# samedii/perceptor

Measured on AMD Instinct MI355X. Metric: denoising steps/sec (UNet+CLIP-grad) at 512x512 batch 8, higher is better.
Workload: dtype bf16

## Files before the change

perceptor_amd/csrc/attn.hip:

```cpp
#include "common.h"
#include "../../include/perceptor_hip.h"

namespace {

__device__ __forceinline__ int64_t tfrag(int bh, int ntb, int tb, int ks, int db, int lhi, int l31) {
  return ((((((int64_t)bh * ntb + tb) * 2 + ks) * 2 + db) * 2 + lhi) * 32 + l31) * 8;
}

__device__ __forceinline__ int64_t rfrag(int bh, int ntb, int tb, int kk, int lhi, int l31) {
  return ((((((int64_t)bh * ntb + tb) * 4 + kk) * 2 + lhi) * 32 + l31) * 8);
}

template <typename T_>
__global__ __launch_bounds__(256) void qkv_split_kernel(const u16* __restrict__ qkv, u16* __restrict__ q,
                                                        u16* __restrict__ k, u16* __restrict__ vt, int T, int Tp,
                                                        int heads, int order) {
  __shared__ u16 sv[32][72];
  const int tid = threadIdx.x, t0 = blockIdx.x * 32, bh = blockIdx.y;
  const int n = bh / heads, h = bh - n * heads;
  const int C = heads * 64;
  const int qoff = order == 0 ? h * 192 : h * 64;
  const int koff = order == 0 ? h * 192 + 64 : C + h * 64;
  const int voff = order == 0 ? h * 192 + 128 : 2 * C + h * 64;
  const int row = tid >> 3, ch = tid & 7;
  const int t = t0 + row;
  uint4 vq = make_uint4(0, 0, 0, 0), vk = vq, vv = vq;
  if (t < T) {
    const u16* src = qkv + ((int64_t)n * T + t) * 3 * C + ch * 8;
    vq = *(const uint4*)(src + qoff); vk = *(const uint4*)(src + koff); vv = *(const uint4*)(src + voff);
  }
  const int64_t o = rfrag(bh, Tp >> 5, blockIdx.x, ch >> 1, ch & 1, row);
  *(uint4*)(q + o) = vq;
  *(uint4*)(k + o) = vk;
  *(uint4*)(&sv[row][ch * 8]) = vv;
  __syncthreads();
  const int d = tid >> 2, tc = tid & 3, fks = tc >> 1, flhi = tc & 1;
  u16 e[8];
#pragma unroll
  for (int j = 0; j < 8; ++j) e[j] = sv[16 * fks + 4 * flhi + (j & 3) + 8 * (j >> 2)][d];
  uint4 out = make_uint4(e[0] | (e[1] << 16), e[2] | (e[3] << 16), e[4] | (e[5] << 16), e[6] | (e[7] << 16));
  *(uint4*)(vt + tfrag(bh, Tp >> 5, blockIdx.x, fks, d >> 5, flhi, d & 31)) = out;
}

__device__ __forceinline__ void head_xcd_remap(int& bx, int& bh) {
// ... 420 lines not shown
    u16* ovp = okp + C;
#pragma unroll
    for (int g = 0; g < 4; ++g) {
      *(uint2*)(okp + 8 * g) = pack4<T_>(dk0[4 * g], dk0[4 * g + 1], dk0[4 * g + 2], dk0[4 * g + 3]);
      *(uint2*)(okp + 32 + 8 * g) = pack4<T_>(dk1[4 * g], dk1[4 * g + 1], dk1[4 * g + 2], dk1[4 * g + 3]);
      *(uint2*)(ovp + 8 * g) = pack4<T_>(dv0[4 * g], dv0[4 * g + 1], dv0[4 * g + 2], dv0[4 * g + 3]);
      *(uint2*)(ovp + 32 + 8 * g) = pack4<T_>(dv1[4 * g], dv1[4 * g + 1], dv1[4 * g + 2], dv1[4 * g + 3]);
    }
  }
}

template <typename T_>
__global__ __launch_bounds__(64) void vit_attn_bwd_kernel(const u16* __restrict__ q, const u16* __restrict__ k, const u16* __restrict__ v,
                                                          const u16* __restrict__ qt, const u16* __restrict__ kt,
                                                          const u16* __restrict__ d_o, const u16* __restrict__ d_ot,
                                                          const float* __restrict__ lse, const float* __restrict__ delta,
                                                          u16* __restrict__ dqkv, int T, int Tp, int heads, float scale) {
  int bx, bh;
  head_xcd_remap(bx, bh);
  if (blockIdx.z == 0) vit_attn_dkdv_body<T_>(q, k, v, qt, d_o, d_ot, lse, delta, dqkv, T, Tp, heads, scale, bx, bh);
  else vit_attn_dq_body<T_>(q, k, v, kt, d_o, lse, delta, dqkv, T, Tp, heads, scale, bx, bh);
}

}

#define VIT_BY_DTYPE(KERN, G, B, ...)                                                             \
  do {                                                                                            \
    if (dtype == PMI_DT_BF16) hipLaunchKernelGGL(KERN<BF16>, G, B, 0, (hipStream_t)s, __VA_ARGS__); \
    else hipLaunchKernelGGL(KERN<F16>, G, B, 0, (hipStream_t)s, __VA_ARGS__);                     \
  } while (0)

extern "C" int pmi_vit_attn_fwd(const void* qkv, void* ws16, float* lse, void* out, int N, int T, int heads, float scale, int dtype,
                                pmi_stream_t s) {
  if (!qkv || !ws16 || !lse || !out || N <= 0 || T <= 0 || heads <= 0) return PMI_ERR_ARG;
  const int Tp = (T + 31) / 32 * 32;
  const int64_t blk = (int64_t)N * heads * Tp * 64;
  u16* w = (u16*)ws16;
  dim3 g(Tp / 32, N * heads);
  VIT_BY_DTYPE(vit_qkv_split_kernel, g, dim3(256), (const u16*)qkv, w, w + blk, w + 2 * blk, w + 3 * blk, w + 4 * blk, w + 5 * blk, T, Tp, heads);
  PMI_CHECK_LAUNCH();
  VIT_BY_DTYPE(vit_attn_fwd_kernel, g, dim3(64), w, w + blk, w + 5 * blk, (u16*)out, lse, T, Tp, heads, scale);
  PMI_CHECK_LAUNCH();
  return PMI_OK;
}

extern "C" int pmi_vit_attn_bwd(const void* ws16, const float* lse, const void* o, const void* dout, void* ws16b, float* delta,
                                void* dqkv, int N, int T, int heads, float scale, int dtype, pmi_stream_t s) {
  if (!ws16 || !lse || !o || !dout || !ws16b || !delta || !dqkv || N <= 0 || T <= 0 || heads <= 0) return PMI_ERR_ARG;
  const int Tp = (T + 31) / 32 * 32;
  const int64_t blk = (int64_t)N * heads * Tp * 64;
  const u16* w = (const u16*)ws16;
  u16* wb = (u16*)ws16b;
  dim3 g(Tp / 32, N * heads);
  VIT_BY_DTYPE(vit_do_prep_kernel, g, dim3(256), (const u16*)dout, (const u16*)o, wb, wb + blk, delta, T, Tp, heads);
  PMI_CHECK_LAUNCH();
  dim3 g2(Tp / 32, N * heads, 2);
  VIT_BY_DTYPE(vit_attn_bwd_kernel, g2, dim3(64), w, w + blk, w + 2 * blk, w + 3 * blk, w + 4 * blk, wb, wb + blk, lse, delta, (u16*)dqkv, T, Tp,
               heads, scale);
  PMI_CHECK_LAUNCH();
  return PMI_OK;
}
```

perceptor_amd/csrc/common.h:

```cpp
#pragma once
#include <type_traits>
#include <hip/hip_runtime.h>
#include <stdint.h>

#define PMI_OK 0
#define PMI_ERR_ARG (-1)
#define PMI_ERR_LAUNCH (-2)

#define PMI_DT_F16 0
#define PMI_DT_BF16 1
#define PMI_DT_F16X2 2

#define PMI_ACT_NONE 0
#define PMI_ACT_RELU 1
#define PMI_ACT_SILU 2
#define PMI_ACT_GELU 3
#define PMI_ACT_QUICKGELU 4
#define PMI_ACT_GEGLU 5

typedef _Float16 f16x8 __attribute__((ext_vector_type(8)));
typedef __bf16 bf16x8 __attribute__((ext_vector_type(8)));
typedef float f32x2 __attribute__((ext_vector_type(2)));
typedef _Float16 f16x2 __attribute__((ext_vector_type(2)));
typedef __bf16 bf16x2 __attribute__((ext_vector_type(2)));
// ... 138 lines not shown
  act_switch(act, [&](auto act_c) __attribute__((always_inline)) {
#pragma unroll
    for (int e = 0; e < N; ++e) v[e] = act_apply(v[e], decltype(act_c)::value);
  });
}

__device__ __forceinline__ float act_grad(float x, int act) {
  switch (act) {
    case PMI_ACT_RELU: return x > 0.f ? 1.f : 0.f;
    case PMI_ACT_SILU: { const float s = 1.f / (1.f + __expf(-x)); return s * (1.f + x * (1.f - s)); }
    case PMI_ACT_GELU: return 0.5f * (1.f + fast_erff(x * 0.70710678118654752f)) + x * 0.3989422804014327f * __expf(-0.5f * x * x);
    case PMI_ACT_QUICKGELU: { const float s = 1.f / (1.f + __expf(-1.702f * x)); return s * (1.f + 1.702f * x * (1.f - s)); }
    default: return 1.f;
  }
}

__device__ __forceinline__ float wave_sum(float v) {
#pragma unroll
  for (int o = 32; o > 0; o >>= 1) v += __shfl_xor(v, o);
  return v;
}
__device__ __forceinline__ float wave_max(float v) {
#pragma unroll
  for (int o = 32; o > 0; o >>= 1) v = fmaxf(v, __shfl_xor(v, o));
  return v;
}

__device__ __forceinline__ int xcd_remap(int bid, int nwg) {
  const int q = nwg >> 3, r = nwg & 7, xcd = bid & 7, idx = bid >> 3;
  const int base = xcd < r ? xcd * (q + 1) : r * (q + 1) + (xcd - r) * q;
  return base + idx;
}

#define PMI_CHECK_LAUNCH()                                   \
  do {                                                       \
    hipError_t e__ = hipGetLastError();                      \
    if (e__ != hipSuccess) return PMI_ERR_LAUNCH;            \
  } while (0)
```

perceptor_amd/csrc/gemm_wd.hip:

```cpp
#include "common.h"
#include "../../include/perceptor_hip.h"

namespace {

template <typename T, int MB, bool TWO = false, int NWV = 8, bool CONV = false>
__global__ __launch_bounds__(NWV * 64, 2) void gemm_wd_kernel(const pmi_igemm_args a) {
  constexpr int TM = 16 * MB, BN = NWV * 32, BK = 128, NT = NWV * 64;
  constexpr int ROW = 2 * BK + 32;
  constexpr int TILE = TM * ROW;
  constexpr int NPI = (TM * 16 + NT - 1) / NT;
  constexpr int HIMG = TM * (BN * 2 + 16);
  __shared__ __attribute__((aligned(16))) char smem[2 * TILE > 2 * HIMG ? 2 * TILE : 2 * HIMG];

  const int tid = threadIdx.x, lane = tid & 63;
  const int wid = __builtin_amdgcn_readfirstlane(tid >> 6);
#ifdef PMI_STAMPS
#define GSTAMP(k) do { if (tid == 0 && a.reserved == 77 && a.splitk <= 1) ((long long*)a.ws)[(int64_t)blockIdx.x * 8 + (k)] = (long long)wall_clock64(); } while (0)
#else
#define GSTAMP(k) do {} while (0)
#endif
  GSTAMP(0);
  const int tiles_n = (a.N + BN - 1) / BN, tiles_m = (a.M + TM - 1) / TM;
  const int logical = xcd_remap(blockIdx.x, tiles_m * tiles_n);
  const bool mfast = (int64_t)a.M <= (int64_t)a.N;
  const int tm = mfast ? logical % tiles_m : logical / tiles_n, tn = mfast ? logical / tiles_m : logical % tiles_n;
  const int m0 = tm * TM, n0 = tn * BN;
  const int nch_all = (a.K + BK - 1) / BK;
  int c0 = 0, nch = nch_all;
  if (a.splitk > 1) {
    const int per = (nch_all + a.splitk - 1) / a.splitk;
    c0 = blockIdx.z * per;
    nch = min(per, nch_all - c0);
  }

  const int rows = min(TM, a.M - m0);
  const int K0 = TWO ? a.C0 : a.K;
  const int64_t mb_ = CONV ? 0 : m0, mr_ = CONV ? a.M : rows;
  const __amdgpu_buffer_rsrc_t rsrc_a = make_rsrc((const u16*)a.A0 + mb_ * a.lda0, ((mr_ - 1) * a.lda0 + K0) * 2);
// ... 84 lines not shown
  for (int mb = 0; mb < MB; ++mb) xf[mb] = *(const uint4*)(smem + frag0 + mb * 16 * ROW);

  for (int chunk = 0; chunk < nch; ++chunk) {
    const char* const pb = smem + (chunk & 1) * TILE;
    char* const pn = smem + ((chunk + 1) & 1) * TILE;
    const bool more2 = chunk + 2 < nch;
#pragma unroll
    for (int s = 0; s < 4; ++s) {
      load_w((s + 3) & 3, chunk * 4 + s + 3);
      if (s == 2) store_tile(pn);
      if (s == 3) {
        load_tile(more2 ? chunk + 2 : chunk, more2);
        __syncthreads();
      }
      __builtin_amdgcn_sched_barrier(0);
      const char* const nb = (s < 3 ? pb + (s + 1) * 64 : pn) + frag0;
#pragma unroll
      for (int mb = 0; mb < MB; ++mb) {
        acc[mb][0] = T::mfma16(wq[s][0], xf[mb], acc[mb][0]);
        acc[mb][1] = T::mfma16(wq[s][1], xf[mb], acc[mb][1]);
        xf[mb] = *(const uint4*)(nb + mb * 16 * ROW);
      }
#pragma unroll
      for (int mb = 0; mb < MB; ++mb) {
        __builtin_amdgcn_sched_group_barrier(0x008, 2, 0);
        __builtin_amdgcn_sched_group_barrier(0x100, 1, 0);
      }
      __builtin_amdgcn_sched_barrier(0);
    }
  }
  __syncthreads();
  GSTAMP(2);

  const bool raw = a.splitk > 1;
  if (a.act == PMI_ACT_GEGLU) {
    constexpr int GROW = (BN / 2) * 2 + 16;
    const int cl = wid * 16 + 4 * (lane >> 4);
    float4 bv = make_float4(0.f, 0.f, 0.f, 0.f), bg = bv;
    if (a.bias && wave_live) { bv = *(const float4*)(a.bias + n0 + wid * 32 + 4 * (lane >> 4)); bg = *(const float4*)(a.bias + n0 + wid * 32 + 16 + 4 * (lane >> 4)); }
#pragma unroll
    for (int mb = 0; mb < MB; ++mb) {
      const f32x4 cv = acc[mb][0], cg = acc[mb][1];
      float v[4] = {cv[0] * a.alpha + bv.x, cv[1] * a.alpha + bv.y, cv[2] * a.alpha + bv.z, cv[3] * a.alpha + bv.w};
      const float g[4] = {cg[0] * a.alpha + bg.x, cg[1] * a.alpha + bg.y, cg[2] * a.alpha + bg.z, cg[3] * a.alpha + bg.w};
#pragma unroll
      for (int e = 0; e < 4; ++e) v[e] *= act_apply(g[e], PMI_ACT_GELU);
      *(uint2*)(smem + (mb * 16 + (lane & 15)) * GROW + cl * 2) = pack4<T>(v[0], v[1], v[2], v[3]);
    }
    __syncthreads();
    const int gc8 = tid % (BN / 16), grow = tid / (BN / 16);
    const int nh = a.N >> 1, nh0 = n0 >> 1;
#pragma unroll
    for (int j = 0; j < (TM + 31) / 32; ++j) {
      const int r = grow + 32 * j, m = m0 + r;
      if (r >= TM || m >= a.M || nh0 + gc8 * 8 >= nh) continue;
      *(uint4*)((u16*)a.D + (int64_t)m * a.ldd + nh0 + gc8 * 8) = *(const uint4*)(smem + r * GROW + gc8 * 16);
    }
    GSTAMP(3);
    return;
  }
  if (!raw && !a.out_f32 && !(a.R && a.res_f32)) {
    constexpr int HROW = BN * 2 + 16;
    static_assert(2 * TM * HROW <= 160 * 1024, "the two 16-bit epilogue images (output, pre-activation) must fit the LDS");
    act_switch(a.act, [&](auto act_c) __attribute__((always_inline)) {
      constexpr int ACT = decltype(act_c)::value;
#pragma unroll
// ... 79 lines not shown
      const int m = m0 + mb * 16 + (lane & 15);
      if (m >= a.M) continue;
      const f32x4 c = acc[mb][cb];
      if (raw) {
        *(float4*)(Dslab + (int64_t)m * a.N + n) = make_float4(c[0], c[1], c[2], c[3]);
        continue;
      }
      float v[4] = {c[0] * a.alpha + bv.x, c[1] * a.alpha + bv.y, c[2] * a.alpha + bv.z, c[3] * a.alpha + bv.w};
#pragma unroll
      for (int e = 0; e < 4; ++e) v[e] = act_apply(v[e], ACT);
      if (a.R) {
        if (a.res_f32) {
          const float4 rr = *(const float4*)((const float*)a.R + (int64_t)m * a.ldr + n);
          v[0] += rr.x; v[1] += rr.y; v[2] += rr.z; v[3] += rr.w;
        } else {
          const uint2 rr = *(const uint2*)((const u16*)a.R + (int64_t)m * a.ldr + n);
          v[0] += T::to_f((u16)(rr.x & 0xffff)); v[1] += T::to_f((u16)(rr.x >> 16));
          v[2] += T::to_f((u16)(rr.y & 0xffff)); v[3] += T::to_f((u16)(rr.y >> 16));
        }
      }
      if (a.out_f32) *(float4*)((float*)a.D + (int64_t)m * a.ldd + n) = make_float4(v[0], v[1], v[2], v[3]);
      else *(uint2*)((u16*)a.D + (int64_t)m * a.ldd + n) = pack4<T>(v[0], v[1], v[2], v[3]);
    }
  }
  });
  GSTAMP(3);
}

static int g_few_wgs = 128;

template <typename T>
int launch(const pmi_igemm_args& a, hipStream_t s, int mb) {
  const int tm = 16 * mb;
  const bool few = a.splitk <= 1 && (long)((a.M + 127) / 128) * ((a.N + 255) / 256) < g_few_wgs && !a.D2 && !a.aux && a.act != PMI_ACT_GEGLU;
  const bool half_tail = (a.N % 256) != 0 && (a.N % 256) <= 128 && a.N < 1024;
  if (a.N < 256 || few || half_tail) {
    const dim3 g4(((a.M + 127) / 128) * ((a.N + 127) / 128), 1, a.splitk > 1 ? a.splitk : 1);
    if (a.taps == 9) {
      if (a.A1) hipLaunchKernelGGL((gemm_wd_kernel<T, 8, true, 4, true>), g4, dim3(256), 0, s, a);
      else hipLaunchKernelGGL((gemm_wd_kernel<T, 8, false, 4, true>), g4, dim3(256), 0, s, a);
    } else if (a.A1) hipLaunchKernelGGL((gemm_wd_kernel<T, 8, true, 4>), g4, dim3(256), 0, s, a);
    else hipLaunchKernelGGL((gemm_wd_kernel<T, 8, false, 4>), g4, dim3(256), 0, s, a);
    PMI_CHECK_LAUNCH();
    return PMI_OK;
  }
  const dim3 grid(((a.M + tm - 1) / tm) * ((a.N + 255) / 256), 1, a.splitk > 1 ? a.splitk : 1);
  if (a.taps == 9) {
    if (a.A1) hipLaunchKernelGGL((gemm_wd_kernel<T, 8, true, 8, true>), grid, dim3(512), 0, s, a);
    else hipLaunchKernelGGL((gemm_wd_kernel<T, 8, false, 8, true>), grid, dim3(512), 0, s, a);
  } else if (a.A1) hipLaunchKernelGGL((gemm_wd_kernel<T, 8, true>), grid, dim3(512), 0, s, a);
  else if (mb == 9) hipLaunchKernelGGL((gemm_wd_kernel<T, 9>), grid, dim3(512), 0, s, a);
  else hipLaunchKernelGGL((gemm_wd_kernel<T, 8>), grid, dim3(512), 0, s, a);
  PMI_CHECK_LAUNCH();
  return PMI_OK;
}

}

void pmi_gemm_wd_few_wgs(int v) { g_few_wgs = v; }

int pmi_gemm_wd_tile_rows(const pmi_igemm_args* a, int splitk) {
  if (a->A1 || a->taps == 9 || a->N < 256 || ((a->N % 256) != 0 && (a->N % 256) <= 128 && a->N < 1024)) return 128;
  if (splitk <= 1 && (long)((a->M + 127) / 128) * ((a->N + 255) / 256) < g_few_wgs && !a->D2 && !a->aux && a->act != PMI_ACT_GEGLU) return 128;
  int best = 8;
  long best_cost = -1;
  for (int mb = 8; mb <= 9; ++mb) {
    const long wgs = (long)((a->M + 16 * mb - 1) / (16 * mb)) * ((a->N + 255) / 256) * (splitk > 1 ? splitk : 1);
    const long cost = ((wgs + 255) / 256) * mb;
    if (best_cost < 0 || cost < best_cost) { best_cost = cost; best = mb; }
  }
  return 16 * best;
}

int pmi_igemm_halo_allowed(void);

extern "C" int pmi_gemm_wd_eligible(const pmi_igemm_args* a) {
  if (!a->Bf || (a->taps != 1 && a->taps != 9) || a->up || a->stride != 1 || a->batch > 1) return 0;
  if (a->taps == 9) {
    if ((a->C0 % 128) || (a->A1 ? (a->C1 <= 0 || (a->C1 % 128)) : a->C1 != 0) || a->D2 || a->aux || a->act == PMI_ACT_GEGLU || a->split_in) return 0;
    if (a->H <= 0 || a->W <= 0 || a->H >= 0x4000 || a->W >= 0x4000 || a->Hin != a->H || a->Win != a->W || (a->M % (a->H * a->W))) return 0;
    if (a->K != 9 * (a->C0 + a->C1) || (int64_t)a->M * (a->lda0 > a->lda1 ? a->lda0 : a->lda1) * 2 >= ((int64_t)1 << 31)) return 0;
    if (pmi_igemm_halo_allowed() && pmi_conv3x3_halo_config(a) >= 0) return 0;
    if (a->M < 512) return 0;
  } else {
    if (a->A1 ? (a->C1 <= 0 || (a->C0 % 128) || (a->C1 % 32) || a->splitk > 1 || a->D2 || a->aux || a->act == PMI_ACT_GEGLU) : a->C1 != 0) return 0;
    if (a->K != a->C0 + a->C1) return 0;
  }
  if (a->nbias && (a->taps != 9 || a->splitk == 1)) return 0;
  if (a->res_up && (a->taps != 9 || a->splitk == 1)) return 0;
  if (a->stats || a->pro_a || a->split_out) return 0;
  if ((a->K % 32) || (a->N % 32) || a->M < 64) return 0;
  if (a->N < 256 && a->N != 128) return 0;
  if ((a->N % 256) && a->N < 1024) {
    const int tail = a->N % 256;
    if (tail < 64) return 0;
  }
  if ((a->D2 || a->aux) && (a->out_f32 || a->splitk > 1 || (a->R && a->res_f32))) return 0;
  if (a->act == PMI_ACT_GEGLU && (a->R || a->D2 || a->aux || a->out_f32 || a->splitk > 1)) return 0;
  return 1;
}

int pmi_gemm_wd_launch(const pmi_igemm_args* a, void* stream) {
  hipStream_t s = (hipStream_t)stream;
  const int mb = pmi_gemm_wd_tile_rows(a, a->splitk) / 16;
  return a->dtype == PMI_DT_BF16 ? launch<BF16>(*a, s, mb) : launch<F16>(*a, s, mb);
}
```

perceptor_amd/csrc/igemm.hip:

```cpp
#include <cstdio>
#include <cstdlib>
#include "common.h"
#include "epilogue.h"
#include "../../include/perceptor_hip.h"

namespace {

constexpr int BM = 128, BN = 128, BK = 64;
constexpr int TILE_BYTES = 128 * 128;
constexpr int STAGE_BYTES = 2 * TILE_BYTES;

__device__ __forceinline__ int lds_off(int row, int chunk) { return row * 128 + ((chunk ^ ((row >> 1) & 7)) << 4); }

template <typename T, bool CONV, bool KFAST>
__global__ __launch_bounds__(256, 2) void igemm_kernel(const pmi_igemm_args a) {
  __shared__ __attribute__((aligned(16))) char smem[2 * STAGE_BYTES];

  const int tid = threadIdx.x, lane = tid & 63, wid = tid >> 6;
  const int wr = wid >> 1, wc = wid & 1;
#ifdef PMI_STAMPS
#define GSTAMP(k) do { if (tid == 0 && a.reserved == 77 && a.splitk <= 1) ((long long*)a.ws)[(int64_t)blockIdx.x * 8 + (k)] = (long long)wall_clock64(); } while (0)
#else
#define GSTAMP(k) do {} while (0)
#endif
// ... 554 lines not shown

static int bad_arg(int line) {
  if (getenv("PMI_DEBUG")) fprintf(stderr, "pmi_igemm: argument check at igemm.hip:%d failed\n", line);
  return PMI_ERR_ARG;
}

extern "C" int pmi_igemm(const pmi_igemm_args* a, pmi_stream_t stream) {
  if (!a || !a->A0 || !a->B || !a->D) return bad_arg(__LINE__);
  if (a->M <= 0 || a->N <= 0 || a->K <= 0) return bad_arg(__LINE__);
  if ((a->K & 7) || (a->C0 & 7) || (a->C1 & 7)) return bad_arg(__LINE__);
  if ((a->N & 3) && (a->bias || a->nbias || a->R || a->ldd < ((a->N + 3) & ~3))) return bad_arg(__LINE__);
  if ((a->lda0 & 7) || (a->ldb & 7) || (a->ldd & 3)) return bad_arg(__LINE__);
  if (a->C1 > 0 && (!a->A1 || (a->lda1 & 7))) return bad_arg(__LINE__);
  if (a->taps != 1 && a->taps != 9 && a->taps != 16) return bad_arg(__LINE__);
  if (a->taps == 16 && (a->stride != 2 || a->up || a->res_up || a->Hin != 2 * a->H || a->Win != 2 * a->W)) return bad_arg(__LINE__);
  if (a->stride != 1 && a->stride != 2) return bad_arg(__LINE__);
  if (a->K != a->taps * (a->C0 + a->C1)) return bad_arg(__LINE__);
  if (a->R && (a->ldr & 3)) return bad_arg(__LINE__);
  if (a->split_out && ((a->split_out & 7) || a->split_out > 32 || a->out_f32 || (a->N % a->split_out) || a->batch > 1)) return bad_arg(__LINE__);
  if ((unsigned)a->split_in > 2u) return bad_arg(__LINE__);
  if (a->split_in == 2 && !a->split_out) return bad_arg(__LINE__);
  if (a->nbias && a->hw <= 0) return bad_arg(__LINE__);
  const bool conv = a->taps != 1 || a->up || a->stride == 2;
  if (a->res_up && ((a->H & 1) || (a->W & 1))) return bad_arg(__LINE__);
  if ((conv || a->res_up) && (a->H <= 0 || a->W <= 0 || a->Hin <= 0 || a->Win <= 0 || a->M % (a->H * a->W))) return bad_arg(__LINE__);
  if (a->up && (a->H != 2 * a->Hin || a->W != 2 * a->Win)) return bad_arg(__LINE__);
  if (a->batch > 1 && a->batch_inner <= 0) return bad_arg(__LINE__);
  const int halo = g_allow_halo ? pmi_conv3x3_halo_config(a) : -1;
  if (a->pro_a && (!a->pro_b || halo < 0)) return PMI_ERR_ARG;
  if ((a->split_in == 2 || ((a->split_in || a->split_out) && a->pro_a) || (a->split_out && a->R && a->res_f32)) && halo < 6) return bad_arg(__LINE__);
  if (a->stats && a->stats_p != pmi_igemm_stats_rows(a)) return PMI_ERR_ARG;
  if (a->splitk > 1 && (!a->ws || a->batch > 1 || (halo >= 0 && a->splitk != pmi_conv3x3_wd_splitk(a, halo)) || (a->N & 3) || a->stats)) return PMI_ERR_ARG;
  if (a->act == PMI_ACT_GEGLU && !pmi_gemm_wd_eligible(a)) return bad_arg(__LINE__);
  if ((a->D2 || a->aux) && !pmi_gemm_wd_eligible(a)) return bad_arg(__LINE__);
  if (pmi_gemm_wd_eligible(a) && !((a->nbias || a->res_up) && a->splitk <= 1)) {
    const int rc = pmi_gemm_wd_launch(a, stream);
    if (rc != PMI_OK || a->splitk <= 1 || a->reserved3 == 1) return rc;
    hipStream_t s = (hipStream_t)stream;
    const int64_t work = (int64_t)a->M * (a->N / 4);
    const int blocks = (int)((work + 255) / 256 > 4096 ? 4096 : (work + 255) / 256);
    if (a->dtype == PMI_DT_BF16) hipLaunchKernelGGL(splitk_reduce_kernel<BF16>, dim3(blocks), dim3(256), 0, s, *a);
    else hipLaunchKernelGGL(splitk_reduce_kernel<F16>, dim3(blocks), dim3(256), 0, s, *a);
    PMI_CHECK_LAUNCH();
    return PMI_OK;
  }
  if (halo >= 4) {
    const int rc = pmi_conv3x3_wd_launch(a, halo, stream);
    if (rc != PMI_OK || a->splitk <= 1) return rc;
    hipStream_t s = (hipStream_t)stream;
    const int64_t work = (int64_t)a->M * (a->N / 4);
    const int blocks = (int)((work + 255) / 256 > 4096 ? 4096 : (work + 255) / 256);
    if (a->dtype == PMI_DT_BF16) hipLaunchKernelGGL(splitk_reduce_kernel<BF16>, dim3(blocks), dim3(256), 0, s, *a);
    else hipLaunchKernelGGL(splitk_reduce_kernel<F16>, dim3(blocks), dim3(256), 0, s, *a);
    PMI_CHECK_LAUNCH();
    return PMI_OK;
  }
  if (halo >= 0) return pmi_conv3x3_halo_launch(a, halo, stream);
  hipStream_t s = (hipStream_t)stream;
  return a->dtype == PMI_DT_BF16 ? launch<BF16>(*a, s) : launch<F16>(*a, s);
}

extern "C" int pmi_abi_version(void) { return 1; }
```

perceptor_amd/engine/ops.py:

```python
from __future__ import annotations

import math
import os
import ctypes as C
from typing import Optional

import torch

from .. import _hip
from .._hip import ACT_GEGLU, ACT_NONE, DT_F16X2, IgemmArgs, call, ptr


HALO_ENABLED = True
SPLITK_ENABLED = True
WD_ENABLED = True
GEMM_WD_ENABLED = True
GEMM_WD_CONV = os.environ.get("PMI_GEMM_WD_CONV", "1") != "0"
FLASH_ENABLED = True


def set_halo(enabled: bool) -> None:
    global HALO_ENABLED
    HALO_ENABLED = bool(enabled)
    _hip.lib().pmi_set_option(0, int(enabled))
# ... 408 lines not shown

def geglu_linear(x: torch.Tensor, lin: PackedLinear) -> torch.Tensor:
    dt = lin.dt
    a = IgemmArgs()
    a.taps, a.stride, a.M, a.N, a.K, a.C0, a.batch, a.Bf, a.act = 1, 1, x.shape[0], lin.n_p, lin.K, lin.K, 1, 1, ACT_GEGLU
    if GEMM_WD_ENABLED and not lin.split and lin.n_p % 32 == 0 and lin.K % 32 == 0 and _hip.lib().pmi_gemm_wd_eligible(C.byref(a)):
        return igemm(x, lin, act=ACT_GEGLU)
    f = igemm(x, lin)
    out = _empty((x.shape[0], lin.n_p // 2), f.dtype, f.device)
    call("pmi_geglu", ptr(f), ptr(out), x.shape[0], lin.n_p // 2, 1, dt)
    return out


def interleave_geglu(weight: torch.Tensor, bias: Optional[torch.Tensor]):
    f = weight.shape[0] // 2
    assert f % 16 == 0
    idx = torch.arange(f).view(-1, 16)
    perm = torch.cat([idx, idx + f], dim=1).flatten()
    return weight[perm].contiguous(), (bias[perm].contiguous() if bias is not None else None)


def fused_mlp_epilogues(lin: PackedLinear, m: int) -> bool:
    if not (GEMM_WD_ENABLED and lin.taps == 1 and not lin.split and lin.n_p % 256 == 0 and lin.K % 128 == 0 and m >= 64):
        return False
    a = IgemmArgs()
    a.taps, a.stride, a.M, a.N, a.K, a.C0, a.batch, a.batch_inner, a.hw = 1, 1, m, lin.n_p, lin.K, lin.K, 1, 1, 1
    a.lda0, a.ldb, a.ldd, a.dtype, a.alpha = lin.K, lin.K, lin.n_p, lin.dt, 1.0
    a.Bf, a.D2 = 1, 1
    if SPLITK_ENABLED and _hip.lib().pmi_igemm_splitk(C.byref(a)) > 1:
        return False
    return bool(_hip.lib().pmi_gemm_wd_eligible(C.byref(a)))


def bgemm(A: torch.Tensor, B: torch.Tensor, D: torch.Tensor, *, M: int, N: int, K: int, lda: int, ldb: int, ldd: int,
          batch: int, batch_inner: int, sA, sB, sD, dt: int, alpha: float = 1.0, a_off: int = 0, b_off: int = 0, d_off: int = 0):
    a = IgemmArgs()
    es = A.element_size()
    a.A0 = A.data_ptr() + a_off * es
    a.B = B.data_ptr() + b_off * B.element_size()
    a.D = D.data_ptr() + d_off * D.element_size()
    a.M, a.N, a.K, a.C0, a.C1 = M, N, K, K, 0
    a.lda0, a.ldb, a.ldd = lda, ldb, ldd
    a.taps, a.stride, a.hw, a.alpha = 1, 1, 1, alpha
    a.out_f32 = int(D.dtype == torch.float32)
    a.batch, a.batch_inner = batch, batch_inner
    a.sA_o, a.sA_i = sA
    a.sB_o, a.sB_i = sB
    a.sD_o, a.sD_i = sD
    a.dtype = dt
    if GEMM_TRACE is not None:
        e0, e1 = torch.cuda.Event(enable_timing=True), torch.cuda.Event(enable_timing=True)
        e0.record()
        call("pmi_igemm", C.byref(a))
        e1.record()
        GEMM_TRACE.append((f"bgemm M={M} N={N} K={K} batch={batch}", 2.0 * M * N * K * batch, e0, e1))
        return D
    call("pmi_igemm", C.byref(a))
    return D


def _gn_coeffs(x, x1, gamma, beta, groups, dt, film, film_ld, eps):
    n, h, w, _ = x.shape
    c0 = logical_c(x, dt)
    c1 = logical_c(x1, dt) if x1 is not None else 0
    c, hw, dev = c0 + c1, h * w, x.device
    ca = _empty((n, c), torch.float32, dev)
# ... 492 lines not shown
```

perceptor_amd/engine/vit.py:

```python
from __future__ import annotations

from typing import Dict, Tuple

import torch

from .. import _hip
from .._hip import ACT_GELU, ACT_NONE, ACT_QUICKGELU, call, ptr
from ..transforms.resize import resize as _resize, resize_backward as _resize_backward
from . import ops
from .ops import PackedLinear

CLIP_MEAN = (0.48145466, 0.4578275, 0.40821073)
CLIP_STD = (0.26862954, 0.26130258, 0.27577711)

VIT_CONFIGS = {
    "ViT-B-32": (224, 32, 768, 12, 12, 512),
    "ViT-B-16": (224, 16, 768, 12, 12, 512),
    "ViT-L-14": (224, 14, 1024, 24, 16, 768),
    "ViT-H-14": (224, 14, 1280, 32, 16, 1024),
}


def vit_state_dict_shapes(cfg) -> Dict[str, Tuple[int, ...]]:
    res, patch, width, layers, heads, out = cfg
# ... 131 lines not shown
        call("pmi_transpose_16", src.data_ptr() + off * src.element_size(), ptr(out), rows, cols, ld, s_o, s_i, inner, batch)
        return out

    @torch.no_grad()
    def forward(self, images: torch.Tensor, save: bool = False, features: bool = False):
        if not images.is_cuda:
            raise RuntimeError("VitEngine runs on a HIP device only (no CPU fallback)")
        res, patch, width, layers, heads, out = self.cfg
        dt, dev = self.dt, self.device
        tdt = _hip.TORCH_DTYPE[dt]
        n = images.shape[0]
        g = res // patch
        t = g * g + 1
        m = n * t
        tp = (t + 7) // 8 * 8
        d = width // heads
        resized = _resize(images, (res, res))
        col = torch.empty((n * g * g, self.kp), dtype=tdt, device=dev)
        call("pmi_patchify", ptr(resized), ptr(self.mean), ptr(self.std), ptr(col), n, res, patch, self.kp, 0, dt)
        pe = ops.igemm(col, self.conv1.fwd, out_f32=True)
        x0 = torch.empty((n, t, width), dtype=torch.float32, device=dev)
        call("pmi_vit_assemble", ptr(pe), ptr(self.cls), ptr(self.pos), ptr(x0), n, t, width, 0)
        _, x, mr_pre = self._ln(x0, width, self.ln_pre, m, width, want16=False, want32=True)
        sv = dict(in_hw=tuple(images.shape[2:]), n=n, x0=x0, mr_pre=mr_pre, layers=[]) if save else None
        scale = float(d) ** -0.5
        fuse = width % 256 == 0 and width <= 2048
        nxt = None
        for bi, blk in enumerate(self.blocks):
            if nxt is None:
                h, _, mr1 = self._ln(x, width, blk["ln1"], m, width)
            else:
                h, mr1 = nxt
                nxt = None
            qkv = ops.igemm(h, blk["qkv"].fwd)
            a = torch.empty((m, width), dtype=tdt, device=dev)
            fused = d == 64
            if fused:
                tp32 = (t + 31) // 32 * 32
                aws = torch.empty((6, n * heads, tp32, 64), dtype=tdt, device=dev)
                lse = torch.empty((n * heads, tp32), dtype=torch.float32, device=dev)
                call("pmi_vit_attn_fwd", ptr(qkv), ptr(aws), ptr(lse), ptr(a), n, t, heads, scale, dt)
                p = None
            else:
                s = torch.empty((n * heads, t, tp), dtype=torch.float32, device=dev)
                ops.bgemm(qkv, qkv, s, M=t, N=t, K=d, lda=3 * width, ldb=3 * width, ldd=tp, batch=n * heads, batch_inner=heads,
                          sA=(t * 3 * width, d), sB=(t * 3 * width, d), sD=(heads * t * tp, t * tp), dt=dt, b_off=width)
                p = torch.empty((n * heads, t, tp), dtype=tdt, device=dev)
                call("pmi_softmax_fwd", ptr(s), ptr(p), n * heads * t, t, tp, tp, scale, dt)
                vt = self._transpose(qkv, 2 * width, t, d, 3 * width, t * 3 * width, d, heads, n * heads)
                ops.bgemm(p, vt, a, M=t, N=d, K=tp, lda=tp, ldb=tp, ldd=width, batch=n * heads, batch_inner=heads,
                          sA=(heads * t * tp, t * tp), sB=(heads * d * tp, d * tp), sD=(t * width, d), dt=dt)
                aws = lse = None
            x_mid = ops.igemm(a, blk["out"].fwd, residual=x, out_f32=True)
            h2, _, mr2 = self._ln(x_mid, width, blk["ln2"], m, width)
            if ops.fused_mlp_epilogues(blk["fc"].fwd, m):
                hpre = torch.empty((m, blk["fc"].fwd.n_p), dtype=tdt, device=dev) if save else None
                hact = ops.igemm(h2, blk["fc"].fwd, act=self.act, pre_out=hpre)
            else:
                hpre = ops.igemm(h2, blk["fc"].fwd)
                hact = torch.empty_like(hpre)
                call("pmi_act_fwd", ptr(hpre), ptr(hact), hpre.numel(), self.act, dt)
            last = bi + 1 == len(self.blocks)
            x_out = ops.igemm(hact, blk["pr"].fwd, residual=x_mid, out_f32=True, defer_reduce=fuse and not last)
            if isinstance(x_out, tuple):
                x_out, hn, mrn = self._ln_slabs(x_out, blk["pr"].fwd.b, x_mid, self.blocks[bi + 1]["ln1"], m, width)
                nxt = (hn, mrn)
            if save:
                sv["layers"].append(dict(x_in=x, mr1=mr1, qkv=qkv if not fused else None, p=p, aws=aws, lse=lse, a=a if fused else None,
                                         x_mid=x_mid, mr2=mr2, hpre=hpre))
            x = x_out
        y16, y32, mr_post = self._ln(x, t * width, self.ln_post, n, width, want32=features)
        emb = ops.igemm(y16, self.proj.fwd, out_f32=True)
        if save:
            sv.update(x_final=x, mr_post=mr_post)
            self.saved = sv
        emb = emb[:, :out] if emb.shape[1] != out else emb
        return (emb, x.view(n, t, width), y32) if features else emb

    @torch.no_grad()
    def backward(self, d_emb: torch.Tensor) -> torch.Tensor:
        sv = self.saved
        if sv is None:
            raise RuntimeError("call forward(images, save=True) before backward()")
        res, patch, width, layers, heads, out = self.cfg
        dt, dev = self.dt, self.device
        tdt = _hip.TORCH_DTYPE[dt]
        n = sv["n"]
        g = res // patch
        t = g * g + 1
        m = n * t
        tp = (t + 7) // 8 * 8
        d = width // heads
        scale = float(d) ** -0.5
        d16 = torch.empty((n, out), dtype=tdt, device=dev)
        d_emb = d_emb.contiguous()
        call("pmi_cast_f32_to_16", ptr(d_emb), ptr(d16), n * out, ACT_NONE, dt)
        dy_post = ops.igemm(d16, self.proj.bwd, out_f32=True)
        g32 = torch.zeros((m, width), dtype=torch.float32, device=dev)
        g16 = torch.zeros((m, width), dtype=tdt, device=dev)
        self._ln_bwd(dy_post, dy_post.shape[1], sv["x_final"], self.ln_post, sv["mr_post"], None, n, width, row_stride=t, g32=g32, g16=g16)
        for blk, L in zip(reversed(self.blocks), reversed(sv["layers"])):
            if ops.fused_mlp_epilogues(blk["pr"].bwd, m):
                dh = ops.igemm(g16, blk["pr"].bwd, act_grad_of=L["hpre"], act_grad=self.act)
            else:
                dh = ops.igemm(g16, blk["pr"].bwd)
                call("pmi_act_bwd", ptr(dh), ptr(L["hpre"]), ptr(dh), dh.numel(), self.act, dt)
            fuse = width % 256 == 0 and width <= 2048
            dln2 = ops.igemm(dh, blk["fc"].bwd, out_f32=True, defer_reduce=fuse)
            gm32, gm16 = self._ln_bwd_any(dln2, L["x_mid"], blk["ln2"], L["mr2"], g32, m, width)
            da = ops.igemm(gm16, blk["out"].bwd)
            w3 = 3 * width
            dqkv = torch.empty((m, w3), dtype=tdt, device=dev)
            if L["aws"] is not None:
                tp32 = (t + 31) // 32 * 32
                bws = torch.empty((2, n * heads, tp32, 64), dtype=tdt, device=dev)
                delta = torch.empty((n * heads, tp32), dtype=torch.float32, device=dev)
                call("pmi_vit_attn_bwd", ptr(L["aws"]), ptr(L["lse"]), ptr(L["a"]), ptr(da), ptr(bws), ptr(delta), ptr(dqkv),
                     n, t, heads, scale, dt)
            else:
                qkv, p = L["qkv"], L["p"]
                dp = torch.empty((n * heads, t, tp), dtype=torch.float32, device=dev)
                ops.bgemm(da, qkv, dp, M=t, N=t, K=d, lda=width, ldb=w3, ldd=tp, batch=n * heads, batch_inner=heads,
                          sA=(t * width, d), sB=(t * w3, d), sD=(heads * t * tp, t * tp), dt=dt, b_off=2 * width)
                ds = torch.empty((n * heads, t, tp), dtype=tdt, device=dev)
                call("pmi_softmax_bwd", ptr(dp), ptr(p), ptr(ds), n * heads * t, t, tp, tp, scale, dt)
                pt = self._transpose(p, 0, t, t, tp, heads * t * tp, t * tp, heads, n * heads)
                dot = self._transpose(da, 0, t, d, width, t * width, d, heads, n * heads)
                ops.bgemm(pt, dot, dqkv, M=t, N=d, K=tp, lda=tp, ldb=tp, ldd=w3, batch=n * heads, batch_inner=heads,
                          sA=(heads * t * tp, t * tp), sB=(heads * d * tp, d * tp), sD=(t * w3, d), dt=dt, d_off=2 * width)
                kt = self._transpose(qkv, width, t, d, w3, t * w3, d, heads, n * heads)
                ops.bgemm(ds, kt, dqkv, M=t, N=d, K=tp, lda=tp, ldb=tp, ldd=w3, batch=n * heads, batch_inner=heads,
                          sA=(heads * t * tp, t * tp), sB=(heads * d * tp, d * tp), sD=(t * w3, d), dt=dt)
                dst = self._transpose(ds, 0, t, t, tp, heads * t * tp, t * tp, heads, n * heads)
                qt = self._transpose(qkv, 0, t, d, w3, t * w3, d, heads, n * heads)
                ops.bgemm(dst, qt, dqkv, M=t, N=d, K=tp, lda=tp, ldb=tp, ldd=w3, batch=n * heads, batch_inner=heads,
                          sA=(heads * t * tp, t * tp), sB=(heads * d * tp, d * tp), sD=(t * w3, d), dt=dt, d_off=width)
            dln1 = ops.igemm(dqkv, blk["qkv"].bwd, out_f32=True, defer_reduce=fuse)
            g32, g16 = self._ln_bwd_any(dln1, L["x_in"], blk["ln1"], L["mr1"], gm32, m, width)
        _, g0 = self._ln_bwd(g32, width, sv["x0"], self.ln_pre, sv["mr_pre"], None, m, width, want32=False)
        dcol = torch.empty((n * (t - 1), self.kp), dtype=torch.float32, device=dev)
        ops.bgemm(g0, self.conv1.bwd.w, dcol, M=t - 1, N=self.kp, K=width, lda=width, ldb=width, ldd=self.kp, batch=n, batch_inner=1,
                  sA=(t * width, 0), sB=(0, 0), sD=((t - 1) * self.kp, 0), dt=dt, a_off=width)
        dres = torch.empty((n, 3, res, res), dtype=torch.float32, device=dev)
        call("pmi_unpatchify", ptr(dcol), ptr(self.std), ptr(dres), n, res, patch, self.kp, 1.0 / self.gscale)
        self.saved = None
        return _resize_backward(dres, sv["in_hw"])
```

Before: 24.99.

## Fuse attention operand packing into QKV and out-proj GEMM epilogues

Adds an ATTN epilogue mode to the weights-direct GEMM. In this mode the GEMM writes Q/K/V straight into the fragment-packed layouts (row fragments and transposed fragments) that the fused ViT attention kernels read. In backward, the out-projection GEMM likewise emits the packed dO operands and computes the delta dot product with O, so the separate qkv_split and do_prep kernels are skipped. This removes the intermediate qkv/da round trip through memory and two kernel launches per layer. In exchange the GEMM epilogue gains scattered stores, padding handling and more shared-memory traffic, and the path only applies when head dim is 64 and the GEMM is eligible.

```diff
diff --git a/perceptor_amd/csrc/attn.hip b/perceptor_amd/csrc/attn.hip
--- a/perceptor_amd/csrc/attn.hip
+++ b/perceptor_amd/csrc/attn.hip
@@ -3,13 +3,6 @@
 
 namespace {
 
-__device__ __forceinline__ int64_t tfrag(int bh, int ntb, int tb, int ks, int db, int lhi, int l31) {
-  return ((((((int64_t)bh * ntb + tb) * 2 + ks) * 2 + db) * 2 + lhi) * 32 + l31) * 8;
-}
-
-__device__ __forceinline__ int64_t rfrag(int bh, int ntb, int tb, int kk, int lhi, int l31) {
-  return ((((((int64_t)bh * ntb + tb) * 4 + kk) * 2 + lhi) * 32 + l31) * 8);
-}
 
 template <typename T_>
 __global__ __launch_bounds__(256) void qkv_split_kernel(const u16* __restrict__ qkv, u16* __restrict__ q,
@@ -496,13 +489,15 @@
 
 extern "C" int pmi_vit_attn_fwd(const void* qkv, void* ws16, float* lse, void* out, int N, int T, int heads, float scale, int dtype,
                                 pmi_stream_t s) {
-  if (!qkv || !ws16 || !lse || !out || N <= 0 || T <= 0 || heads <= 0) return PMI_ERR_ARG;
+  if (!ws16 || !lse || !out || N <= 0 || T <= 0 || heads <= 0) return PMI_ERR_ARG;
   const int Tp = (T + 31) / 32 * 32;
   const int64_t blk = (int64_t)N * heads * Tp * 64;
   u16* w = (u16*)ws16;
   dim3 g(Tp / 32, N * heads);
-  VIT_BY_DTYPE(vit_qkv_split_kernel, g, dim3(256), (const u16*)qkv, w, w + blk, w + 2 * blk, w + 3 * blk, w + 4 * blk, w + 5 * blk, T, Tp, heads);
-  PMI_CHECK_LAUNCH();
+  if (qkv) {
+    VIT_BY_DTYPE(vit_qkv_split_kernel, g, dim3(256), (const u16*)qkv, w, w + blk, w + 2 * blk, w + 3 * blk, w + 4 * blk, w + 5 * blk, T, Tp, heads);
+    PMI_CHECK_LAUNCH();
+  }
   VIT_BY_DTYPE(vit_attn_fwd_kernel, g, dim3(64), w, w + blk, w + 5 * blk, (u16*)out, lse, T, Tp, heads, scale);
   PMI_CHECK_LAUNCH();
   return PMI_OK;
@@ -510,14 +505,16 @@
 
 extern "C" int pmi_vit_attn_bwd(const void* ws16, const float* lse, const void* o, const void* dout, void* ws16b, float* delta,
                                 void* dqkv, int N, int T, int heads, float scale, int dtype, pmi_stream_t s) {
-  if (!ws16 || !lse || !o || !dout || !ws16b || !delta || !dqkv || N <= 0 || T <= 0 || heads <= 0) return PMI_ERR_ARG;
+  if (!ws16 || !lse || (dout && !o) || !ws16b || !delta || !dqkv || N <= 0 || T <= 0 || heads <= 0) return PMI_ERR_ARG;
   const int Tp = (T + 31) / 32 * 32;
   const int64_t blk = (int64_t)N * heads * Tp * 64;
   const u16* w = (const u16*)ws16;
   u16* wb = (u16*)ws16b;
   dim3 g(Tp / 32, N * heads);
-  VIT_BY_DTYPE(vit_do_prep_kernel, g, dim3(256), (const u16*)dout, (const u16*)o, wb, wb + blk, delta, T, Tp, heads);
-  PMI_CHECK_LAUNCH();
+  if (dout) {
+    VIT_BY_DTYPE(vit_do_prep_kernel, g, dim3(256), (const u16*)dout, (const u16*)o, wb, wb + blk, delta, T, Tp, heads);
+    PMI_CHECK_LAUNCH();
+  }
   dim3 g2(Tp / 32, N * heads, 2);
   VIT_BY_DTYPE(vit_attn_bwd_kernel, g2, dim3(64), w, w + blk, w + 2 * blk, w + 3 * blk, w + 4 * blk, wb, wb + blk, lse, delta, (u16*)dqkv, T, Tp,
                heads, scale);
diff --git a/perceptor_amd/csrc/common.h b/perceptor_amd/csrc/common.h
--- a/perceptor_amd/csrc/common.h
+++ b/perceptor_amd/csrc/common.h
@@ -194,6 +194,14 @@
   return base + idx;
 }
 
+__device__ __forceinline__ int64_t tfrag(int bh, int ntb, int tb, int ks, int db, int lhi, int l31) {
+  return ((((((int64_t)bh * ntb + tb) * 2 + ks) * 2 + db) * 2 + lhi) * 32 + l31) * 8;
+}
+
+__device__ __forceinline__ int64_t rfrag(int bh, int ntb, int tb, int kk, int lhi, int l31) {
+  return ((((((int64_t)bh * ntb + tb) * 4 + kk) * 2 + lhi) * 32 + l31) * 8);
+}
+
 #define PMI_CHECK_LAUNCH()                                   \
   do {                                                       \
     hipError_t e__ = hipGetLastError();                      \
diff --git a/perceptor_amd/csrc/gemm_wd.hip b/perceptor_amd/csrc/gemm_wd.hip
--- a/perceptor_amd/csrc/gemm_wd.hip
+++ b/perceptor_amd/csrc/gemm_wd.hip
@@ -3,7 +3,97 @@
 
 namespace {
 
-template <typename T, int MB, bool TWO = false, int NWV = 8, bool CONV = false>
+template <typename T, int MB, int NWV>
+__device__ __forceinline__ void attn_operand_epilogue(const pmi_igemm_args& a, const f32x4 (&acc)[MB][2], char* smem, int m0, int n0, int tid,
+                                                      bool wave_live) {
+  constexpr int TM = 16 * MB, BN = NWV * 32, NT = NWV * 64, HROW = BN * 2 + 16, HT = BN / 64;
+  const int lane = tid & 63, wid = tid >> 6;
+  const int Tk = a.hw, Tp = (Tk + 31) & ~31, ntb = Tp >> 5;
+  const int C = a.ldd, heads = C >> 6, nw = a.N / C;
+  const int64_t blk = (int64_t)(a.M / Tk) * heads * Tp * 64;
+  u16* const D = (u16*)a.D;
+  float* const delta = (float*)a.D2;
+#pragma unroll
+  for (int cb = 0; cb < 2; ++cb) {
+    const int nl = wid * 32 + cb * 16 + 4 * (lane >> 4);
+    float4 bv = make_float4(0.f, 0.f, 0.f, 0.f);
+    if (a.bias && wave_live) bv = *(const float4*)(a.bias + n0 + nl);
+#pragma unroll
+    for (int mb = 0; mb < MB; ++mb) {
+      const f32x4 c = acc[mb][cb];
+      *(uint2*)(smem + (mb * 16 + (lane & 15)) * HROW + nl * 2) =
+          pack4<T>(c[0] * a.alpha + bv.x, c[1] * a.alpha + bv.y, c[2] * a.alpha + bv.z, c[3] * a.alpha + bv.w);
+    }
+  }
+  const int ch = tid & 7;
+  uint4 ov[MB];
+#pragma unroll
+  for (int j = 0; j < MB; ++j) {
+    const int u = (tid >> 3) + (NT / 8) * j, r = u % TM, hd = u / TM, m = m0 + r;
+    ov[j] = make_uint4(0, 0, 0, 0);
+    if (delta && m < a.M && n0 + hd * 64 < a.N) ov[j] = *(const uint4*)((const u16*)a.R + (int64_t)m * a.ldr + n0 + hd * 64 + ch * 8);
+  }
+  __syncthreads();
+#pragma unroll
+  for (int j = 0; j < MB; ++j) {
+    const int u = (tid >> 3) + (NT / 8) * j, r = u % TM, hd = u / TM, m = m0 + r;
+    const bool live = m < a.M && n0 + hd * 64 < a.N;
+    const uint4 v = *(const uint4*)(smem + r * HROW + (hd * 8 + ch) * 16);
+    const int img = m / Tk, t = m - img * Tk;
+    const int hg = (n0 >> 6) + hd, w = hg / heads, bh = img * heads + (hg - w * heads);
+    if (live) *(uint4*)(D + w * blk + rfrag(bh, ntb, t >> 5, ch >> 1, ch & 1, t & 31)) = v;
+    if (delta) {
+      float fa[8], fb[8], p = 0.f;
+      unpack8<T>(v, fa); unpack8<T>(ov[j], fb);
+#pragma unroll
+      for (int e = 0; e < 8; ++e) p += fa[e] * fb[e];
+      p += __shfl_xor(p, 1); p += __shfl_xor(p, 2); p += __shfl_xor(p, 4);
+      if (live && ch == 0) delta[(int64_t)bh * Tp + t] = p;
+    }
+  }
+  const int rows = min(TM, a.M - m0), ml = m0 + rows - 1;
+  const int img_lo = m0 / Tk, img_hi = ml / Tk, t_hi = ml - img_hi * Tk;
+  const int P_lo = img_lo * Tp + (m0 - img_lo * Tk), P_hi = img_hi * Tp + (t_hi == Tk - 1 ? Tp - 1 : t_hi);
+  const int nP = P_hi - P_lo + 1;
+  if (nP != rows) {
+    for (int u = tid >> 3; u < nP * HT; u += NT / 8) {
+      const int hd = u / nP, P = P_lo + (u - hd * nP);
+      const int img = P / Tp, t = P - img * Tp;
+      if (t < Tk || n0 + hd * 64 >= a.N) continue;
+      const int hg = (n0 >> 6) + hd, w = hg / heads, bh = img * heads + (hg - w * heads);
+      *(uint4*)(D + w * blk + rfrag(bh, ntb, t >> 5, ch >> 1, ch & 1, t & 31)) = make_uint4(0, 0, 0, 0);
+      if (delta && ch == 0) delta[(int64_t)bh * Tp + t] = 0.f;
+    }
+  }
+  const int col = tid % BN;
+  if (n0 + col >= a.N) return;
+  const int hg = (n0 + col) >> 6, w = hg / heads, h = hg - w * heads, d = (n0 + col) & 63;
+  const int G_lo = P_lo >> 4, nG = (P_hi >> 4) - G_lo + 1;
+  for (int gl = tid / BN; gl < 2 * nG; gl += NT / BN) {
+    const int lhi = gl & 1, Pg = (G_lo + (gl >> 1)) * 16;
+    const int img = Pg / Tp, tg = Pg - img * Tp;
+    const int rbase = img * Tk + tg - m0;
+    u16 e[8];
+    unsigned own = 0;
+#pragma unroll
+    for (int j = 0; j < 8; ++j) {
+      const int o = 4 * lhi + (j & 3) + 8 * (j >> 2), P = Pg + o;
+      const bool mine = P >= P_lo && P <= P_hi;
+      own |= (unsigned)mine << j;
+      e[j] = (mine && tg + o < Tk) ? *(const u16*)(smem + (rbase + o) * HROW + col * 2) : (u16)0;
+    }
+    u16* const dst = D + (nw + w) * blk + tfrag(img * heads + h, ntb, tg >> 5, (tg >> 4) & 1, d >> 5, lhi, d & 31);
+    if (own == 0xffu) {
+      *(uint4*)dst = make_uint4(e[0] | (e[1] << 16), e[2] | (e[3] << 16), e[4] | (e[5] << 16), e[6] | (e[7] << 16));
+    } else {
+#pragma unroll
+      for (int j = 0; j < 8; ++j)
+        if ((own >> j) & 1u) dst[j] = e[j];
+    }
+  }
+}
+
+template <typename T, int MB, bool TWO = false, int NWV = 8, bool CONV = false, bool ATTN = false>
 __global__ __launch_bounds__(NWV * 64, 2) void gemm_wd_kernel(const pmi_igemm_args a) {
   constexpr int TM = 16 * MB, BN = NWV * 32, BK = 128, NT = NWV * 64;
   constexpr int ROW = 2 * BK + 32;
@@ -154,6 +244,11 @@
   __syncthreads();
   GSTAMP(2);
 
+  if constexpr (ATTN) {
+    attn_operand_epilogue<T, MB, NWV>(a, acc, smem, m0, n0, tid, wave_live);
+    GSTAMP(3);
+    return;
+  }
   const bool raw = a.splitk > 1;
   if (a.act == PMI_ACT_GEGLU) {
     constexpr int GROW = (BN / 2) * 2 + 16;
@@ -299,11 +394,13 @@
 template <typename T>
 int launch(const pmi_igemm_args& a, hipStream_t s, int mb) {
   const int tm = 16 * mb;
-  const bool few = a.splitk <= 1 && (long)((a.M + 127) / 128) * ((a.N + 255) / 256) < g_few_wgs && !a.D2 && !a.aux && a.act != PMI_ACT_GEGLU;
+  const bool attn = a.reserved3 == 2;
+  const bool few = a.splitk <= 1 && (long)((a.M + 127) / 128) * ((a.N + 255) / 256) < g_few_wgs && (attn || (!a.D2 && !a.aux)) && a.act != PMI_ACT_GEGLU;
   const bool half_tail = (a.N % 256) != 0 && (a.N % 256) <= 128 && a.N < 1024;
   if (a.N < 256 || few || half_tail) {
     const dim3 g4(((a.M + 127) / 128) * ((a.N + 127) / 128), 1, a.splitk > 1 ? a.splitk : 1);
-    if (a.taps == 9) {
+    if (attn) hipLaunchKernelGGL((gemm_wd_kernel<T, 8, false, 4, false, true>), g4, dim3(256), 0, s, a);
+    else if (a.taps == 9) {
       if (a.A1) hipLaunchKernelGGL((gemm_wd_kernel<T, 8, true, 4, true>), g4, dim3(256), 0, s, a);
       else hipLaunchKernelGGL((gemm_wd_kernel<T, 8, false, 4, true>), g4, dim3(256), 0, s, a);
     } else if (a.A1) hipLaunchKernelGGL((gemm_wd_kernel<T, 8, true, 4>), g4, dim3(256), 0, s, a);
@@ -312,7 +409,10 @@
     return PMI_OK;
   }
   const dim3 grid(((a.M + tm - 1) / tm) * ((a.N + 255) / 256), 1, a.splitk > 1 ? a.splitk : 1);
-  if (a.taps == 9) {
+  if (attn) {
+    if (mb == 9) hipLaunchKernelGGL((gemm_wd_kernel<T, 9, false, 8, false, true>), grid, dim3(512), 0, s, a);
+    else hipLaunchKernelGGL((gemm_wd_kernel<T, 8, false, 8, false, true>), grid, dim3(512), 0, s, a);
+  } else if (a.taps == 9) {
     if (a.A1) hipLaunchKernelGGL((gemm_wd_kernel<T, 8, true, 8, true>), grid, dim3(512), 0, s, a);
     else hipLaunchKernelGGL((gemm_wd_kernel<T, 8, false, 8, true>), grid, dim3(512), 0, s, a);
   } else if (a.A1) hipLaunchKernelGGL((gemm_wd_kernel<T, 8, true>), grid, dim3(512), 0, s, a);
@@ -328,7 +428,7 @@
 
 int pmi_gemm_wd_tile_rows(const pmi_igemm_args* a, int splitk) {
   if (a->A1 || a->taps == 9 || a->N < 256 || ((a->N % 256) != 0 && (a->N % 256) <= 128 && a->N < 1024)) return 128;
-  if (splitk <= 1 && (long)((a->M + 127) / 128) * ((a->N + 255) / 256) < g_few_wgs && !a->D2 && !a->aux && a->act != PMI_ACT_GEGLU) return 128;
+  if (splitk <= 1 && (long)((a->M + 127) / 128) * ((a->N + 255) / 256) < g_few_wgs && (a->reserved3 == 2 || (!a->D2 && !a->aux)) && a->act != PMI_ACT_GEGLU) return 128;
   int best = 8;
   long best_cost = -1;
   for (int mb = 8; mb <= 9; ++mb) {
@@ -343,6 +443,12 @@
 
 extern "C" int pmi_gemm_wd_eligible(const pmi_igemm_args* a) {
   if (!a->Bf || (a->taps != 1 && a->taps != 9) || a->up || a->stride != 1 || a->batch > 1) return 0;
+  const bool attn = a->reserved3 == 2;
+  if (attn) {
+    if (a->taps != 1 || a->A1 || a->aux || a->out_f32 || a->splitk > 1 || a->act != PMI_ACT_NONE || a->split_in || a->split_out || a->nbias) return 0;
+    if (a->hw <= 0 || (a->M % a->hw) || a->ldd <= 0 || (a->ldd % 64) || (a->N % a->ldd)) return 0;
+    if (a->D2 ? (!a->R || a->res_f32 || a->N != a->ldd || (a->ldr & 7)) : a->R != nullptr) return 0;
+  }
   if (a->taps == 9) {
     if ((a->C0 % 128) || (a->A1 ? (a->C1 <= 0 || (a->C1 % 128)) : a->C1 != 0) || a->D2 || a->aux || a->act == PMI_ACT_GEGLU || a->split_in) return 0;
     if (a->H <= 0 || a->W <= 0 || a->H >= 0x4000 || a->W >= 0x4000 || a->Hin != a->H || a->Win != a->W || (a->M % (a->H * a->W))) return 0;
@@ -356,13 +462,13 @@
   if (a->nbias && (a->taps != 9 || a->splitk == 1)) return 0;
   if (a->res_up && (a->taps != 9 || a->splitk == 1)) return 0;
   if (a->stats || a->pro_a || a->split_out) return 0;
-  if ((a->K % 32) || (a->N % 32) || a->M < 64) return 0;
+  if ((a->K % 32) || (a->N % 32) || (a->M < 64 && !attn)) return 0;
   if (a->N < 256 && a->N != 128) return 0;
   if ((a->N % 256) && a->N < 1024) {
     const int tail = a->N % 256;
     if (tail < 64) return 0;
   }
-  if ((a->D2 || a->aux) && (a->out_f32 || a->splitk > 1 || (a->R && a->res_f32))) return 0;
+  if (!attn && (a->D2 || a->aux) && (a->out_f32 || a->splitk > 1 || (a->R && a->res_f32))) return 0;
   if (a->act == PMI_ACT_GEGLU && (a->R || a->D2 || a->aux || a->out_f32 || a->splitk > 1)) return 0;
   return 1;
 }
diff --git a/perceptor_amd/csrc/igemm.hip b/perceptor_amd/csrc/igemm.hip
--- a/perceptor_amd/csrc/igemm.hip
+++ b/perceptor_amd/csrc/igemm.hip
@@ -610,6 +610,7 @@
   if (a->stats && a->stats_p != pmi_igemm_stats_rows(a)) return PMI_ERR_ARG;
   if (a->splitk > 1 && (!a->ws || a->batch > 1 || (halo >= 0 && a->splitk != pmi_conv3x3_wd_splitk(a, halo)) || (a->N & 3) || a->stats)) return PMI_ERR_ARG;
   if (a->act == PMI_ACT_GEGLU && !pmi_gemm_wd_eligible(a)) return bad_arg(__LINE__);
+  if (a->reserved3 == 2 && !pmi_gemm_wd_eligible(a)) return bad_arg(__LINE__);
   if ((a->D2 || a->aux) && !pmi_gemm_wd_eligible(a)) return bad_arg(__LINE__);
   if (pmi_gemm_wd_eligible(a) && !((a->nbias || a->res_up) && a->splitk <= 1)) {
     const int rc = pmi_gemm_wd_launch(a, stream);
diff --git a/perceptor_amd/engine/ops.py b/perceptor_amd/engine/ops.py
--- a/perceptor_amd/engine/ops.py
+++ b/perceptor_amd/engine/ops.py
@@ -464,6 +464,40 @@
     return bool(_hip.lib().pmi_gemm_wd_eligible(C.byref(a)))
 
 
+def attn_operands_fused(lin: PackedLinear, m: int) -> bool:
+    if not (GEMM_WD_ENABLED and lin.taps == 1 and not lin.split and lin.n_p % 64 == 0 and lin.K % 32 == 0) or DEBUG_WS is not None or GEMM_TRACE is not None:
+        return False
+    a = IgemmArgs()
+    a.taps, a.stride, a.M, a.N, a.K, a.C0, a.batch, a.batch_inner, a.hw = 1, 1, m, lin.n_p, lin.K, lin.K, 1, 1, 1
+    a.lda0, a.ldb, a.ldd, a.dtype, a.alpha = lin.K, lin.K, lin.n_p, lin.dt, 1.0
+    a.Bf = 1
+    if not _hip.lib().pmi_gemm_wd_eligible(C.byref(a)):
+        return False
+    return not (SPLITK_ENABLED and _hip.lib().pmi_igemm_splitk(C.byref(a)) > 1)
+
+
+def igemm_attn_operands(a0: torch.Tensor, lin: PackedLinear, n: int, t: int, width: int, o: Optional[torch.Tensor] = None):
+    dt = lin.dt
+    m = a0.shape[0]
+    assert a0.ndim == 2 and m == n * t and a0.shape[1] == lin.cin_p and width % 64 == 0 and lin.n_p % width == 0
+    heads, nw, tp32 = width // 64, lin.n_p // width, (t + 31) // 32 * 32
+    buf = _empty((2 * nw, n * heads, tp32, 64), _hip.TORCH_DTYPE[dt], a0.device)
+    delta = _empty((n * heads, tp32), torch.float32, a0.device) if o is not None else None
+    a = IgemmArgs()
+    a.A0, a.B, a.Bf, a.bias, a.D = ptr(a0), ptr(lin.w), ptr(lin.frag_gemm()), ptr(lin.b), ptr(buf)
+    a.M, a.N, a.K, a.C0 = m, lin.n_p, lin.K, lin.K
+    a.lda0, a.ldb, a.ldd = a0.stride(0), lin.K, width
+    a.taps, a.stride, a.alpha, a.batch, a.batch_inner, a.dtype = 1, 1, 1.0, 1, 1, dt
+    a.hw, a.reserved3 = t, 2
+    if o is not None:
+        assert o.shape == (m, width) and o.dtype == buf.dtype
+        a.R, a.ldr, a.D2 = ptr(o), o.stride(0), ptr(delta)
+    if not _hip.lib().pmi_gemm_wd_eligible(C.byref(a)):
+        raise RuntimeError(f"igemm_attn_operands: the weights-direct GEMM does not take M={m} N={lin.n_p} K={lin.K} (no other kernel has this epilogue)")
+    call("pmi_igemm", C.byref(a))
+    return buf, delta
+
+
 def bgemm(A: torch.Tensor, B: torch.Tensor, D: torch.Tensor, *, M: int, N: int, K: int, lda: int, ldb: int, ldd: int,
           batch: int, batch_inner: int, sA, sB, sD, dt: int, alpha: float = 1.0, a_off: int = 0, b_off: int = 0, d_off: int = 0):
     a = IgemmArgs()
diff --git a/perceptor_amd/engine/vit.py b/perceptor_amd/engine/vit.py
--- a/perceptor_amd/engine/vit.py
+++ b/perceptor_amd/engine/vit.py
@@ -187,16 +187,21 @@
             else:
                 h, mr1 = nxt
                 nxt = None
-            qkv = ops.igemm(h, blk["qkv"].fwd)
             a = torch.empty((m, width), dtype=tdt, device=dev)
             fused = d == 64
             if fused:
                 tp32 = (t + 31) // 32 * 32
-                aws = torch.empty((6, n * heads, tp32, 64), dtype=tdt, device=dev)
                 lse = torch.empty((n * heads, tp32), dtype=torch.float32, device=dev)
+                if ops.attn_operands_fused(blk["qkv"].fwd, m):
+                    qkv = None
+                    aws, _ = ops.igemm_attn_operands(h, blk["qkv"].fwd, n, t, width)
+                else:
+                    qkv = ops.igemm(h, blk["qkv"].fwd)
+                    aws = torch.empty((6, n * heads, tp32, 64), dtype=tdt, device=dev)
                 call("pmi_vit_attn_fwd", ptr(qkv), ptr(aws), ptr(lse), ptr(a), n, t, heads, scale, dt)
                 p = None
             else:
+                qkv = ops.igemm(h, blk["qkv"].fwd)
                 s = torch.empty((n * heads, t, tp), dtype=torch.float32, device=dev)
                 ops.bgemm(qkv, qkv, s, M=t, N=t, K=d, lda=3 * width, ldb=3 * width, ldd=tp, batch=n * heads, batch_inner=heads,
                           sA=(t * 3 * width, d), sB=(t * 3 * width, d), sD=(heads * t * tp, t * tp), dt=dt, b_off=width)
@@ -263,16 +268,21 @@
             fuse = width % 256 == 0 and width <= 2048
             dln2 = ops.igemm(dh, blk["fc"].bwd, out_f32=True, defer_reduce=fuse)
             gm32, gm16 = self._ln_bwd_any(dln2, L["x_mid"], blk["ln2"], L["mr2"], g32, m, width)
-            da = ops.igemm(gm16, blk["out"].bwd)
             w3 = 3 * width
             dqkv = torch.empty((m, w3), dtype=tdt, device=dev)
             if L["aws"] is not None:
                 tp32 = (t + 31) // 32 * 32
-                bws = torch.empty((2, n * heads, tp32, 64), dtype=tdt, device=dev)
-                delta = torch.empty((n * heads, tp32), dtype=torch.float32, device=dev)
+                if ops.attn_operands_fused(blk["out"].bwd, m):
+                    da = None
+                    bws, delta = ops.igemm_attn_operands(gm16, blk["out"].bwd, n, t, width, o=L["a"])
+                else:
+                    da = ops.igemm(gm16, blk["out"].bwd)
+                    bws = torch.empty((2, n * heads, tp32, 64), dtype=tdt, device=dev)
+                    delta = torch.empty((n * heads, tp32), dtype=torch.float32, device=dev)
                 call("pmi_vit_attn_bwd", ptr(L["aws"]), ptr(L["lse"]), ptr(L["a"]), ptr(da), ptr(bws), ptr(delta), ptr(dqkv),
                      n, t, heads, scale, dt)
             else:
+                da = ops.igemm(gm16, blk["out"].bwd)
                 qkv, p = L["qkv"], L["p"]
                 dp = torch.empty((n * heads, t, tp), dtype=torch.float32, device=dev)
                 ops.bgemm(da, qkv, dp, M=t, N=t, K=d, lda=width, ldb=w3, ldd=tp, batch=n * heads, batch_inner=heads,
```

After: 24.99. No clear change (-0.0%).
